# seungju-k1m/Distributed_RL

Hardware: NVIDIA H100
Metric: learner transitions/sec (sample+target+prio-update) (higher is better)
Workload: dtype f32

## Files before the change

distributed_rl_b200/csrc/gemm.cu:

```cuda
#include "common.cuh"
#include "hopper.cuh"
#include "operand_image.cuh"

namespace b2rl {
namespace gemm {

using namespace sm90;

constexpr int TM = 128, TN = 256, KC = image::KC;
constexpr int A_TILE = TM * 128, B_TILE = TN * 128;
constexpr int STAGE = 2 * A_TILE + 2 * B_TILE;
constexpr int STAGES = 2;
constexpr int CONSUMERS = 256;
constexpr int THREADS = CONSUMERS + 32;

template <bool TRANSPOSE>
__global__ void __launch_bounds__(256)
k_split_pack(const float* __restrict__ src, int src_rows, int src_cols, int64_t src_ld, int tile_rows,
             float* __restrict__ out, int rows_pad, int k_chunks, int row_off, int kc_off) {
  const int kc = blockIdx.y, row0 = blockIdx.x * 32;
  const int r = threadIdx.x >> 3, unit = threadIdx.x & 7;
  const int row = row0 + r;
  float v[4];
  if (TRANSPOSE) {
    __shared__ float tile[32][33];
    const int lane = threadIdx.x & 31, w = threadIdx.x >> 5;
#pragma unroll
    for (int j = 0; j < 4; ++j) {
      const int k = kc * KC + w * 4 + j, c = row0 + lane;
      tile[w * 4 + j][lane] = (k < src_rows && c < src_cols) ? src[(int64_t)k * src_ld + c] : 0.0f;
    }
    __syncthreads();
#pragma unroll
    for (int e = 0; e < 4; ++e) v[e] = tile[unit * 4 + e][r];
  } else {
    const int k = kc * KC + unit * 4;
    const float* p = src + (int64_t)row * src_ld + k;
    if (row < src_rows && k + 3 < src_cols && ((reinterpret_cast<uintptr_t>(p) & 15) == 0)) {
      const float4 q = *reinterpret_cast<const float4*>(p);
      v[0] = q.x; v[1] = q.y; v[2] = q.z; v[3] = q.w;
    } else {
#pragma unroll
      for (int e = 0; e < 4; ++e) v[e] = (row < src_rows && k + e < src_cols) ? p[e] : 0.0f;
    }
  }
  const int irow = row_off + row, ikc = kc_off + kc;
  if (irow >= rows_pad) return;
  image::store_unit(out, image::offset(irow, ikc, unit, tile_rows, rows_pad), image::term_stride(k_chunks, rows_pad), v);
}

constexpr int ACT_PAD = 1;

template <bool TRANSPOSE>
__global__ void __launch_bounds__(256)
k_pack_act_nhwc(const float* __restrict__ y, int B, int HW, int C, int relu, float* __restrict__ out,
                int rows_pad, int k_chunks) {
  extern __shared__ float s_act[];
  const int K = C * HW;
  if (!TRANSPOSE) {
    const int b = blockIdx.x;
    const int ld = C + ACT_PAD;
    const uint32_t magic_c = (uint32_t)((0x100000000ull + C - 1) / C);
    const uint32_t magic_hw = (uint32_t)((0x100000000ull + HW - 1) / HW);
    if (b < B) {
      const float* src = y + (int64_t)b * K;
      for (int i = threadIdx.x; i < K; i += 256) {
        float v = src[i];
        if (relu) v = fmaxf(v, 0.0f);
        const int hw = (int)__umulhi((uint32_t)i, magic_c);
        s_act[hw * ld + (i - hw * C)] = v;
      }
    }
    __syncthreads();
    const int64_t ts = image::term_stride(k_chunks, rows_pad);
    for (int w = threadIdx.x; w < k_chunks * 8; w += 256) {
      const int kc = w >> 3, unit = w & 7;
      const int f0 = kc * KC + unit * 4;
      int c = (int)__umulhi((uint32_t)f0, magic_hw), hw = f0 - c * HW;
      float v[4];
#pragma unroll
      for (int e = 0; e < 4; ++e) {
        v[e] = (b < B && f0 + e < K) ? s_act[hw * ld + c] : 0.0f;
        if (++hw == HW) { hw = 0; ++c; }
      }
      image::store_unit(out, image::offset(b, kc, unit, TM, rows_pad), ts, v);
    }
  } else {
    const int kc = blockIdx.x, hw = blockIdx.y;
    const int ld = C + ACT_PAD;
    for (int i = threadIdx.x; i < 32 * C; i += 256) {
      const int bb = i / C, c = i - bb * C, b = kc * KC + bb;
      float v = (b < B) ? y[((int64_t)b * HW + hw) * C + c] : 0.0f;
      if (relu) v = fmaxf(v, 0.0f);
      s_act[bb * ld + c] = v;
    }
    __syncthreads();
    const int64_t ts = image::term_stride(k_chunks, rows_pad);
    for (int w = threadIdx.x; w < C * 8; w += 256) {
      const int c = w >> 3, unit = w & 7;
      float v[4];
#pragma unroll
      for (int e = 0; e < 4; ++e) v[e] = s_act[(unit * 4 + e) * ld + c];
      image::store_unit(out, image::offset(c * HW + hw, kc, unit, TN, rows_pad), ts, v);
    }
  }
}

__global__ void __launch_bounds__(256)
k_pack_zero_rows(float* __restrict__ out, int row0, int rows_pad, int k_chunks, int tile_rows) {
  const int64_t ts = image::term_stride(k_chunks, rows_pad);
  const int n_rows = rows_pad - row0;
  const int64_t total = (int64_t)n_rows * k_chunks * 8;
  const float zero[4] = {0.f, 0.f, 0.f, 0.f};
  for (int64_t w = (int64_t)blockIdx.x * 256 + threadIdx.x; w < total; w += (int64_t)gridDim.x * 256) {
    const int unit = (int)(w & 7);
    const int64_t q = w >> 3;
    const int kc = (int)(q / n_rows), f = row0 + (int)(q - (int64_t)kc * n_rows);
    image::store_unit(out, image::offset(f, kc, unit, tile_rows, rows_pad), ts, zero);
  }
}

__global__ void __launch_bounds__(256)
k_unflatten_relu_mask(const float* __restrict__ gx, int64_t gx_ld, int splits, int64_t split_stride,
                      const float* __restrict__ y, int HW, int C, float* __restrict__ out) {
  extern __shared__ float s_act[];
  const int b = blockIdx.x, K = C * HW;
  const float* gr = gx + (int64_t)b * gx_ld;
  for (int i = threadIdx.x; i < K; i += 256) {
    float v = gr[i];
    for (int z = 1; z < splits; ++z) v += gr[z * split_stride + i];
    s_act[i] = v;
  }
  __syncthreads();
  const float* yr = y + (int64_t)b * K;
  float* o = out + (int64_t)b * K;
  for (int i = threadIdx.x; i < K; i += 256) {
    const int hw = i / C, c = i - hw * C;
    o[i] = (yr[i] > 0.0f) ? s_act[c * HW + hw] : 0.0f;
  }
}

struct Params {
  const float* a;
  const float* b;
  float* c;
  int64_t M, N, ldc;
  int64_t m_tiles, n_tiles, k_chunks;
  int32_t splits;
};

__global__ void __launch_bounds__(THREADS, 1)
k_gemm_tf32x3(const __grid_constant__ Params P) {
  extern __shared__ __align__(1024) uint8_t smem_raw[];
  uint8_t* smem = smem_raw + ((1024u - (sptr(smem_raw) & 1023u)) & 1023u);
  __shared__ __align__(8) uint64_t full[STAGES], empty[STAGES];
  const int warp = threadIdx.x >> 5, lane = threadIdx.x & 31;
  const int64_t mt = blockIdx.x, nt = blockIdx.y;
  const int64_t per = (P.k_chunks + P.splits - 1) / P.splits;
  const int64_t k0 = (int64_t)blockIdx.z * per;
  const int64_t k1 = (k0 + per < P.k_chunks) ? k0 + per : P.k_chunks;
  const int64_t nk = k1 - k0;

  if (threadIdx.x == 0) {
    for (int i = 0; i < STAGES; ++i) { mbar_init(&full[i], 1); mbar_init(&empty[i], CONSUMERS); }
    mbar_init_fence();
  }
  __syncthreads();
  if (nk <= 0) return;

  if (warp == CONSUMERS / 32) {
    if (lane == 0) {
      const int64_t a_term = P.k_chunks * P.m_tiles * (TM * 32);
      const int64_t b_term = P.k_chunks * P.n_tiles * (TN * 32);
      for (int64_t i = 0; i < nk; ++i) {
        const int s = (int)(i % STAGES);
        mbar_wait(&empty[s], ((i / STAGES) & 1) ^ 1);
        const int64_t kc = k0 + i;
        const float* a_hi = P.a + (kc * P.m_tiles + mt) * (TM * 32);
        const float* b_hi = P.b + (kc * P.n_tiles + nt) * (TN * 32);
        uint8_t* st = smem + (size_t)s * STAGE;
        mbar_expect_tx(&full[s], STAGE);
        bulk_g2s(st, a_hi, A_TILE, &full[s]);
        bulk_g2s(st + A_TILE, a_hi + a_term, A_TILE, &full[s]);
        bulk_g2s(st + 2 * A_TILE, b_hi, B_TILE, &full[s]);
        bulk_g2s(st + 2 * A_TILE + B_TILE, b_hi + b_term, B_TILE, &full[s]);
      }
    }
    return;
  }

  const int wg = warp >> 2;
  float acc[128];
  for (int64_t i = 0; i < nk; ++i) {
    const int s = (int)(i % STAGES);
    mbar_wait(&full[s], (i / STAGES) & 1);
    const uint32_t base = sptr(smem + (size_t)s * STAGE);
    const uint32_t a_hi = base + wg * (64 * 128), a_lo = a_hi + A_TILE, b_hi = base + 2 * A_TILE, b_lo = b_hi + B_TILE;
    wg_fence();
#pragma unroll
    for (int ks = 0; ks < 4; ++ks) {
      const uint32_t o = ks * 32;
      mma_tf32_n256(acc, make_desc(a_lo + o), make_desc(b_hi + o), (i | ks) ? 1u : 0u);
      mma_tf32_n256(acc, make_desc(a_hi + o), make_desc(b_lo + o), 1u);
      mma_tf32_n256(acc, make_desc(a_hi + o), make_desc(b_hi + o), 1u);
    }
    wg_commit();
    wg_wait<1>();
    wg_fence_regs(acc);
    if (i > 0) mbar_arrive(&empty[(i - 1) % STAGES]);
  }
  wg_wait<0>();
  wg_fence_regs(acc);
  const int64_t r0 = mt * TM + wg * 64 + (warp & 3) * 16 + (lane >> 2);
  float* cz = P.c + (int64_t)blockIdx.z * P.M * P.ldc;
#pragma unroll
  for (int j = 0; j < TN / 8; ++j) {
    const int64_t n = nt * TN + 8 * j + 2 * (lane & 3);
#pragma unroll
    for (int h = 0; h < 2; ++h) {
      const int64_t m = r0 + 8 * h;
      if (m >= P.M || n >= P.N) continue;
      float* dst = cz + m * P.ldc + n;
      if (n + 1 < P.N) *reinterpret_cast<float2*>(dst) = make_float2(acc[4 * j + 2 * h], acc[4 * j + 2 * h + 1]);
      else dst[0] = acc[4 * j + 2 * h];
    }
  }
}

__global__ void __launch_bounds__(256)
k_splitk_reduce(const float* __restrict__ partial, int splits, int64_t M, int64_t N, int64_t ldc, float* __restrict__ c) {
  const int64_t q = (int64_t)blockIdx.x * blockDim.x + threadIdx.x;
  const int64_t per_row = ldc >> 2;
  if (q >= M * per_row) return;
  const int64_t m = q / per_row, n = (q - m * per_row) << 2;
  if (n >= N) return;
  const int64_t off = m * ldc + n, stride = M * ldc;
  if (n + 3 < N) {
    float4 a = *reinterpret_cast<const float4*>(partial + off);
    for (int z = 1; z < splits; ++z) {
      const float4 b = *reinterpret_cast<const float4*>(partial + z * stride + off);
      a.x += b.x; a.y += b.y; a.z += b.z; a.w += b.w;
    }
    *reinterpret_cast<float4*>(c + off) = a;
  } else {
    for (int e = 0; n + e < N; ++e) {
      float a = partial[off + e];
      for (int z = 1; z < splits; ++z) a += partial[z * stride + off + e];
      c[off + e] = a;
    }
  }
}

}
}

using namespace b2rl;

extern "C" int64_t b2rl_gemm_packed_floats(int64_t rows, int64_t k, int32_t b_role) {
  const int64_t tr = b_role ? gemm::TN : gemm::TM;
  const int64_t rows_pad = (rows + tr - 1) / tr * tr, kc = (k + gemm::KC - 1) / gemm::KC;
  return 2 * rows_pad * kc * gemm::KC;
}

extern "C" int b2rl_gemm_split_pack_into(const float* src_dev, int64_t src_rows, int64_t src_cols, int64_t src_ld,
                                         int32_t transpose, int32_t b_role, float* out_dev, int64_t total_rows,
                                         int64_t total_k, int64_t row_offset, int64_t k_offset, void* stream) {
  B2RL_REQUIRE(src_dev && out_dev, "null argument");
  B2RL_REQUIRE(src_rows >= 1 && src_cols >= 1 && src_ld >= src_cols, "bad shape");
  B2RL_REQUIRE(((uintptr_t)out_dev % 16) == 0, "packed operand must be 16-byte aligned");
  const int64_t rows = transpose ? src_cols : src_rows, k = transpose ? src_rows : src_cols;
  B2RL_REQUIRE(row_offset >= 0 && k_offset >= 0 && row_offset + rows <= total_rows && k_offset + k <= total_k,
               "piece outside the operand");
  B2RL_REQUIRE(row_offset % 32 == 0 && k_offset % gemm::KC == 0, "piece offsets must be multiples of 32");
  B2RL_REQUIRE((rows % 32 == 0 || row_offset + rows == total_rows) && (k % gemm::KC == 0 || k_offset + k == total_k),
               "an inner piece must be a multiple of 32 rows / 32 contraction elements");
  const int tr = b_role ? gemm::TN : gemm::TM;
  const int64_t rows_pad = (total_rows + tr - 1) / tr * tr, kc_total = (total_k + gemm::KC - 1) / gemm::KC;
  B2RL_REQUIRE(rows_pad < (1 << 30) && kc_total <= 65535, "operand too large");
  const int64_t rows_cover = (row_offset + rows == total_rows) ? rows_pad - row_offset : rows;
  const int64_t kc_cover = (k + gemm::KC - 1) / gemm::KC;
  dim3 grid((unsigned)(rows_cover / 32), (unsigned)kc_cover);
  if (transpose)
    gemm::k_split_pack<true><<<grid, 256, 0, (cudaStream_t)stream>>>(src_dev, (int)src_rows, (int)src_cols, src_ld, tr,
                                                                     out_dev, (int)rows_pad, (int)kc_total,
                                                                     (int)row_offset, (int)(k_offset / gemm::KC));
  else
    gemm::k_split_pack<false><<<grid, 256, 0, (cudaStream_t)stream>>>(src_dev, (int)src_rows, (int)src_cols, src_ld, tr,
                                                                      out_dev, (int)rows_pad, (int)kc_total,
                                                                      (int)row_offset, (int)(k_offset / gemm::KC));
  count_launch();
  B2RL_CHECK_LAUNCH();
  return B2RL_OK;
}

extern "C" int b2rl_gemm_split_pack(const float* src_dev, int64_t src_rows, int64_t src_cols, int64_t src_ld,
                                    int32_t transpose, int32_t b_role, float* out_dev, void* stream) {
  const int64_t rows = transpose ? src_cols : src_rows, k = transpose ? src_rows : src_cols;
  return b2rl_gemm_split_pack_into(src_dev, src_rows, src_cols, src_ld, transpose, b_role, out_dev, rows, k, 0, 0, stream);
}

constexpr int64_t MAX_CHUNKS_PER_SPLIT = 32;

static int64_t gemm_splits(int64_t M, int64_t N, int64_t K, int sms) {
  const int64_t tiles = ((M + gemm::TM - 1) / gemm::TM) * ((N + gemm::TN - 1) / gemm::TN);
  const int64_t kc = (K + gemm::KC - 1) / gemm::KC;
  int64_t splits = sms / (tiles > 0 ? tiles : 1);
  if (splits < 1) splits = 1;
  if (splits > kc) splits = kc;
  if (splits * MAX_CHUNKS_PER_SPLIT < kc) splits = (kc + MAX_CHUNKS_PER_SPLIT - 1) / MAX_CHUNKS_PER_SPLIT;
  const int64_t per = (kc + splits - 1) / splits;
  return (kc + per - 1) / per;
}

static int gemm_sms(int* out) {
  int dev = 0;
  B2RL_CUDA(cudaGetDevice(&dev));
  B2RL_CUDA(sm_count(dev, out));
  return B2RL_OK;
}

extern "C" int64_t b2rl_gemm_workspace_floats(int64_t M, int64_t N, int64_t K, int64_t ldc) {
  int sms = 0;
  if (gemm_sms(&sms) != B2RL_OK) return -1;
  const int64_t splits = gemm_splits(M, N, K, sms);
  return splits > 1 ? splits * M * ldc : 0;
}

static int gemm_launch(const float* a_packed_dev, const float* b_packed_dev, float* out, int64_t M, int64_t N,
                       int64_t K, int64_t ldc, int64_t splits, cudaStream_t st) {
  int dev = 0;
  B2RL_CUDA(cudaGetDevice(&dev));
  const size_t smem_bytes = (size_t)gemm::STAGES * gemm::STAGE + 1024;
  B2RL_CUDA(set_max_dynamic_smem<gemm::k_gemm_tf32x3>(dev, smem_bytes));
  gemm::Params P{};
  P.a = a_packed_dev; P.b = b_packed_dev;
  P.c = out;
  P.M = M; P.N = N; P.ldc = ldc;
  P.m_tiles = (M + gemm::TM - 1) / gemm::TM;
  P.n_tiles = (N + gemm::TN - 1) / gemm::TN;
  P.k_chunks = (K + gemm::KC - 1) / gemm::KC;
  P.splits = (int32_t)splits;
  dim3 grid((unsigned)P.m_tiles, (unsigned)P.n_tiles, (unsigned)splits);
  gemm::k_gemm_tf32x3<<<grid, gemm::THREADS, smem_bytes, st>>>(P);
  count_launch();
  B2RL_CHECK_LAUNCH();
  return B2RL_OK;
}

extern "C" int b2rl_gemm_tf32x3_partials(const float* a_packed_dev, const float* b_packed_dev, float* partials_dev,
                                         int64_t M, int64_t N, int64_t K, int64_t ldc, void* stream) {
  B2RL_REQUIRE(a_packed_dev && b_packed_dev && partials_dev, "null argument");
  B2RL_REQUIRE(M >= 1 && N >= 1 && K >= 1 && ldc >= N, "bad shape");
  B2RL_REQUIRE(((uintptr_t)partials_dev % 16) == 0 && (ldc % 4) == 0,
               "partials must be 16-byte aligned with ldc % 4 == 0");
  int sms = 0;
  if (int rc = gemm_sms(&sms)) return rc;
  return gemm_launch(a_packed_dev, b_packed_dev, partials_dev, M, N, K, ldc, gemm_splits(M, N, K, sms),
                     (cudaStream_t)stream);
}

extern "C" int b2rl_gemm_tf32x3(const float* a_packed_dev, const float* b_packed_dev, float* c_dev, int64_t M,
                                int64_t N, int64_t K, int64_t ldc, float* workspace_dev, void* stream) {
  B2RL_REQUIRE(a_packed_dev && b_packed_dev && c_dev, "null argument");
  B2RL_REQUIRE(M >= 1 && N >= 1 && K >= 1 && ldc >= N, "bad shape");
  B2RL_REQUIRE(((uintptr_t)c_dev % 16) == 0 && (ldc % 4) == 0, "C must be 16-byte aligned with ldc % 4 == 0");
  int sms = 0;
  if (int rc = gemm_sms(&sms)) return rc;
  const int64_t splits = gemm_splits(M, N, K, sms);
  B2RL_REQUIRE(splits == 1 || (workspace_dev && ((uintptr_t)workspace_dev % 16) == 0),
               "this shape splits K: pass b2rl_gemm_workspace_floats() floats of 16-byte aligned workspace");
  cudaStream_t st = (cudaStream_t)stream;
  if (int rc = gemm_launch(a_packed_dev, b_packed_dev, splits > 1 ? workspace_dev : c_dev, M, N, K, ldc, splits, st))
    return rc;
  if (splits > 1) {
    const int64_t quads = M * (ldc >> 2);
    gemm::k_splitk_reduce<<<(unsigned)((quads + 255) / 256), 256, 0, st>>>(workspace_dev, (int)splits, M, N, ldc, c_dev);
    count_launch();
    B2RL_CHECK_LAUNCH();
  }
  return B2RL_OK;
}


extern "C" int b2rl_gemm_pack_act_nhwc(const float* y_dev, int64_t B, int64_t HW, int64_t C, int32_t relu, int32_t transpose,
                                       float* out_dev, void* stream) {
  B2RL_REQUIRE(y_dev && out_dev, "null argument");
  B2RL_REQUIRE(B >= 1 && HW >= 1 && C >= 1 && C * HW < (1 << 24) && B < (1 << 24), "bad shape");
  B2RL_REQUIRE(((uintptr_t)out_dev % 16) == 0, "packed operand must be 16-byte aligned");
  const int64_t K = C * HW;
  cudaStream_t st = (cudaStream_t)stream;
  if (!transpose) {
    const int64_t rows_pad = (B + gemm::TM - 1) / gemm::TM * gemm::TM, kc = (K + gemm::KC - 1) / gemm::KC;
    const size_t smem = (size_t)HW * (C + gemm::ACT_PAD) * sizeof(float);
    B2RL_REQUIRE(smem <= 48 * 1024, "activation row too large for the staging tile");
    gemm::k_pack_act_nhwc<false><<<(unsigned)rows_pad, 256, smem, st>>>(y_dev, (int)B, (int)HW, (int)C, relu, out_dev,
                                                                       (int)rows_pad, (int)kc);
    count_launch();
  } else {
    const int64_t rows_pad = (K + gemm::TN - 1) / gemm::TN * gemm::TN, kc = (B + gemm::KC - 1) / gemm::KC;
    const size_t smem = (size_t)32 * (C + gemm::ACT_PAD) * sizeof(float);
    B2RL_REQUIRE(smem <= 48 * 1024 && HW <= 65535, "activation tile too large");
    gemm::k_pack_act_nhwc<true><<<dim3((unsigned)kc, (unsigned)HW), 256, smem, st>>>(y_dev, (int)B, (int)HW, (int)C, relu,
                                                                                    out_dev, (int)rows_pad, (int)kc);
    count_launch();
    if (rows_pad > K) {
      gemm::k_pack_zero_rows<<<64, 256, 0, st>>>(out_dev, (int)K, (int)rows_pad, (int)kc, gemm::TN);
      count_launch();
    }
  }
  B2RL_CHECK_LAUNCH();
  return B2RL_OK;
}

extern "C" int b2rl_unflatten_relu_mask(const float* gx_dev, int64_t gx_ld, int32_t splits, int64_t split_stride,
                                        const float* y_dev, int64_t B, int64_t HW, int64_t C, float* out_dev,
                                        void* stream) {
  B2RL_REQUIRE(gx_dev && y_dev && out_dev, "null argument");
  B2RL_REQUIRE(B >= 1 && HW >= 1 && C >= 1 && gx_ld >= C * HW, "bad shape");
  B2RL_REQUIRE(splits >= 1 && (splits == 1 || split_stride >= B * gx_ld), "bad split-K partials");
  const size_t smem = (size_t)C * HW * sizeof(float);
  B2RL_REQUIRE(smem <= 48 * 1024, "activation row too large for the staging tile");
  gemm::k_unflatten_relu_mask<<<(unsigned)B, 256, smem, (cudaStream_t)stream>>>(gx_dev, gx_ld, splits, split_stride,
                                                                              y_dev, (int)HW, (int)C, out_dev);
  count_launch();
  B2RL_CHECK_LAUNCH();
  return B2RL_OK;
}
```

distributed_rl_b200/csrc/hopper.cuh:

```cuda
#pragma once
#include <stdint.h>

namespace b2rl {
namespace sm90 {

__device__ __forceinline__ uint32_t sptr(const void* p) { return (uint32_t)__cvta_generic_to_shared(p); }
__device__ __forceinline__ void mbar_init(uint64_t* b, uint32_t c) {
  asm volatile("mbarrier.init.shared::cta.b64 [%0], %1;" ::"r"(sptr(b)), "r"(c));
}
__device__ __forceinline__ void mbar_init_fence() {
  asm volatile("fence.mbarrier_init.release.cluster;" ::: "memory");
  asm volatile("fence.proxy.async.shared::cta;" ::: "memory");
}
__device__ __forceinline__ void mbar_expect_tx(uint64_t* b, uint32_t bytes) {
  asm volatile("mbarrier.arrive.expect_tx.shared::cta.b64 _, [%0], %1;" ::"r"(sptr(b)), "r"(bytes) : "memory");
}
__device__ __forceinline__ void mbar_arrive(uint64_t* b) {
  asm volatile("mbarrier.arrive.shared::cta.b64 _, [%0];" ::"r"(sptr(b)) : "memory");
}
__device__ __forceinline__ void mbar_wait(uint64_t* b, uint32_t parity) {
  asm volatile(
      "{\n\t.reg .pred p;\n\t"
      "W_%=:\n\t"
      "mbarrier.try_wait.parity.shared::cta.b64 p, [%0], %1;\n\t"
      "@p bra D_%=;\n\t"
      "bra W_%=;\n\t"
      "D_%=:\n\t}" ::"r"(sptr(b)), "r"(parity) : "memory");
}
__device__ __forceinline__ void bulk_g2s(void* dst, const void* src, uint32_t bytes, uint64_t* bar) {
  asm volatile("cp.async.bulk.shared::cluster.global.mbarrier::complete_tx::bytes [%0], [%1], %2, [%3];" ::"r"(
                   sptr(dst)), "l"(src), "r"(bytes), "r"(sptr(bar)) : "memory");
}
__device__ __forceinline__ void bulk_s2g(void* dst, const void* src, uint32_t bytes) {
  asm volatile("cp.async.bulk.global.shared::cta.bulk_group [%0], [%1], %2;" ::"l"(dst), "r"(sptr(src)), "r"(bytes)
               : "memory");
}
__device__ __forceinline__ void bulk_commit() { asm volatile("cp.async.bulk.commit_group;" ::: "memory"); }
template <int N>
__device__ __forceinline__ void bulk_wait_read() { asm volatile("cp.async.bulk.wait_group.read %0;" ::"n"(N) : "memory"); }
__device__ __forceinline__ void bulk_wait_all() { asm volatile("cp.async.bulk.wait_group 0;" ::: "memory"); }
__device__ __forceinline__ void fence_async_smem() { asm volatile("fence.proxy.async.shared::cta;" ::: "memory"); }
__device__ __forceinline__ void named_sync(int id, int threads) {
  asm volatile("bar.sync %0, %1;" ::"r"(id), "r"(threads) : "memory");
}

__device__ __forceinline__ uint64_t make_desc(uint32_t smem_addr) {
  return (uint64_t)((smem_addr & 0x3FFFFu) >> 4) | (1ull << 16) | ((uint64_t)(1024 >> 4) << 32) | (1ull << 62);
}

__device__ __forceinline__ void wg_fence() { asm volatile("wgmma.fence.sync.aligned;" ::: "memory"); }
__device__ __forceinline__ void wg_commit() { asm volatile("wgmma.commit_group.sync.aligned;" ::: "memory"); }
template <int N>
__device__ __forceinline__ void wg_wait() { asm volatile("wgmma.wait_group.sync.aligned %0;" ::"n"(N) : "memory"); }
template <typename T, int R>
__device__ __forceinline__ void wg_fence_regs(T (&d)[R]) {
#pragma unroll
  for (int i = 0; i < R; ++i) asm volatile("" : "+r"(reinterpret_cast<uint32_t&>(d[i]))::"memory");
}

__device__ __forceinline__ void mma_tf32_n256(float (&d)[128], uint64_t a, uint64_t b, uint32_t accumulate) {
  asm volatile(
      "{\n\t.reg .pred p;\n\tsetp.ne.b32 p, %130, 0;\n\t"
      "wgmma.mma_async.sync.aligned.m64n256k8.f32.tf32.tf32 {%0,%1,%2,%3,%4,%5,%6,%7,%8,%9,%10,%11,%12,%13,%14,%15,%16,%17,%18,%19,%20,%21,%22,%23,%24,%25,%26,%27,%28,%29,%30,%31,%32,%33,%34,%35,%36,%37,%38,%39,%40,%41,%42,%43,%44,%45,%46,%47,%48,%49,%50,%51,%52,%53,%54,%55,%56,%57,%58,%59,%60,%61,%62,%63,%64,%65,%66,%67,%68,%69,%70,%71,%72,%73,%74,%75,%76,%77,%78,%79,%80,%81,%82,%83,%84,%85,%86,%87,%88,%89,%90,%91,%92,%93,%94,%95,%96,%97,%98,%99,%100,%101,%102,%103,%104,%105,%106,%107,%108,%109,%110,%111,%112,%113,%114,%115,%116,%117,%118,%119,%120,%121,%122,%123,%124,%125,%126,%127}, %128, %129, p, 1, 1;\n\t}"
      : "+f"(d[0]), "+f"(d[1]), "+f"(d[2]), "+f"(d[3]), "+f"(d[4]), "+f"(d[5]), "+f"(d[6]), "+f"(d[7]), "+f"(d[8]), "+f"(d[9]), "+f"(d[10]), "+f"(d[11]), "+f"(d[12]), "+f"(d[13]), "+f"(d[14]), "+f"(d[15]), "+f"(d[16]), "+f"(d[17]), "+f"(d[18]), "+f"(d[19]), "+f"(d[20]), "+f"(d[21]), "+f"(d[22]), "+f"(d[23]), "+f"(d[24]), "+f"(d[25]), "+f"(d[26]), "+f"(d[27]), "+f"(d[28]), "+f"(d[29]), "+f"(d[30]), "+f"(d[31]), "+f"(d[32]), "+f"(d[33]), "+f"(d[34]), "+f"(d[35]), "+f"(d[36]), "+f"(d[37]), "+f"(d[38]), "+f"(d[39]), "+f"(d[40]), "+f"(d[41]), "+f"(d[42]), "+f"(d[43]), "+f"(d[44]), "+f"(d[45]), "+f"(d[46]), "+f"(d[47]), "+f"(d[48]), "+f"(d[49]), "+f"(d[50]), "+f"(d[51]), "+f"(d[52]), "+f"(d[53]), "+f"(d[54]), "+f"(d[55]), "+f"(d[56]), "+f"(d[57]), "+f"(d[58]), "+f"(d[59]), "+f"(d[60]), "+f"(d[61]), "+f"(d[62]), "+f"(d[63]), "+f"(d[64]), "+f"(d[65]), "+f"(d[66]), "+f"(d[67]), "+f"(d[68]), "+f"(d[69]), "+f"(d[70]), "+f"(d[71]), "+f"(d[72]), "+f"(d[73]), "+f"(d[74]), "+f"(d[75]), "+f"(d[76]), "+f"(d[77]), "+f"(d[78]), "+f"(d[79]), "+f"(d[80]), "+f"(d[81]), "+f"(d[82]), "+f"(d[83]), "+f"(d[84]), "+f"(d[85]), "+f"(d[86]), "+f"(d[87]), "+f"(d[88]), "+f"(d[89]), "+f"(d[90]), "+f"(d[91]), "+f"(d[92]), "+f"(d[93]), "+f"(d[94]), "+f"(d[95]), "+f"(d[96]), "+f"(d[97]), "+f"(d[98]), "+f"(d[99]), "+f"(d[100]), "+f"(d[101]), "+f"(d[102]), "+f"(d[103]), "+f"(d[104]), "+f"(d[105]), "+f"(d[106]), "+f"(d[107]), "+f"(d[108]), "+f"(d[109]), "+f"(d[110]), "+f"(d[111]), "+f"(d[112]), "+f"(d[113]), "+f"(d[114]), "+f"(d[115]), "+f"(d[116]), "+f"(d[117]), "+f"(d[118]), "+f"(d[119]), "+f"(d[120]), "+f"(d[121]), "+f"(d[122]), "+f"(d[123]), "+f"(d[124]), "+f"(d[125]), "+f"(d[126]), "+f"(d[127])
      : "l"(a), "l"(b), "r"(accumulate));
}

__device__ __forceinline__ void mma_u8s8_n128(int32_t (&d)[64], uint64_t a, uint64_t b, uint32_t accumulate) {
  asm volatile(
      "{\n\t.reg .pred p;\n\tsetp.ne.b32 p, %66, 0;\n\t"
      "wgmma.mma_async.sync.aligned.m64n128k32.s32.u8.s8 {%0,%1,%2,%3,%4,%5,%6,%7,%8,%9,%10,%11,%12,%13,%14,%15,%16,%17,%18,%19,%20,%21,%22,%23,%24,%25,%26,%27,%28,%29,%30,%31,%32,%33,%34,%35,%36,%37,%38,%39,%40,%41,%42,%43,%44,%45,%46,%47,%48,%49,%50,%51,%52,%53,%54,%55,%56,%57,%58,%59,%60,%61,%62,%63}, %64, %65, p;\n\t}"
      : "+r"(d[0]), "+r"(d[1]), "+r"(d[2]), "+r"(d[3]), "+r"(d[4]), "+r"(d[5]), "+r"(d[6]), "+r"(d[7]), "+r"(d[8]), "+r"(d[9]), "+r"(d[10]), "+r"(d[11]), "+r"(d[12]), "+r"(d[13]), "+r"(d[14]), "+r"(d[15]), "+r"(d[16]), "+r"(d[17]), "+r"(d[18]), "+r"(d[19]), "+r"(d[20]), "+r"(d[21]), "+r"(d[22]), "+r"(d[23]), "+r"(d[24]), "+r"(d[25]), "+r"(d[26]), "+r"(d[27]), "+r"(d[28]), "+r"(d[29]), "+r"(d[30]), "+r"(d[31]), "+r"(d[32]), "+r"(d[33]), "+r"(d[34]), "+r"(d[35]), "+r"(d[36]), "+r"(d[37]), "+r"(d[38]), "+r"(d[39]), "+r"(d[40]), "+r"(d[41]), "+r"(d[42]), "+r"(d[43]), "+r"(d[44]), "+r"(d[45]), "+r"(d[46]), "+r"(d[47]), "+r"(d[48]), "+r"(d[49]), "+r"(d[50]), "+r"(d[51]), "+r"(d[52]), "+r"(d[53]), "+r"(d[54]), "+r"(d[55]), "+r"(d[56]), "+r"(d[57]), "+r"(d[58]), "+r"(d[59]), "+r"(d[60]), "+r"(d[61]), "+r"(d[62]), "+r"(d[63])
      : "l"(a), "l"(b), "r"(accumulate));
}

__device__ __forceinline__ void mma_u8s8_n64(int32_t (&d)[32], uint64_t a, uint64_t b, uint32_t accumulate) {
  asm volatile(
      "{\n\t.reg .pred p;\n\tsetp.ne.b32 p, %34, 0;\n\t"
      "wgmma.mma_async.sync.aligned.m64n64k32.s32.u8.s8 {%0,%1,%2,%3,%4,%5,%6,%7,%8,%9,%10,%11,%12,%13,%14,%15,%16,%17,%18,%19,%20,%21,%22,%23,%24,%25,%26,%27,%28,%29,%30,%31}, %32, %33, p;\n\t}"
      : "+r"(d[0]), "+r"(d[1]), "+r"(d[2]), "+r"(d[3]), "+r"(d[4]), "+r"(d[5]), "+r"(d[6]), "+r"(d[7]), "+r"(d[8]), "+r"(d[9]), "+r"(d[10]), "+r"(d[11]), "+r"(d[12]), "+r"(d[13]), "+r"(d[14]), "+r"(d[15]), "+r"(d[16]), "+r"(d[17]), "+r"(d[18]), "+r"(d[19]), "+r"(d[20]), "+r"(d[21]), "+r"(d[22]), "+r"(d[23]), "+r"(d[24]), "+r"(d[25]), "+r"(d[26]), "+r"(d[27]), "+r"(d[28]), "+r"(d[29]), "+r"(d[30]), "+r"(d[31])
      : "l"(a), "l"(b), "r"(accumulate));
}

}
}
```

distributed_rl_b200/csrc/operand_image.cuh:

```cuda
#pragma once
#include <cstdint>

namespace b2rl {
namespace image {

constexpr int KC = 32;

__device__ __forceinline__ void split_tf32(float x, float& hi, float& lo) {
  const uint32_t u = __float_as_uint(x);
  uint32_t h = (u + 0x1000u) & 0xFFFFE000u;
  if ((h & 0x7F800000u) == 0x7F800000u) h = u & 0xFFFFE000u;
  hi = __uint_as_float(h);
  lo = ((u & 0x7F800000u) == 0x7F800000u) ? 0.0f : x - hi;
  if ((u & 0x7F800000u) == 0x7F800000u) hi = x;
}

__host__ __device__ __forceinline__ int64_t term_stride(int k_chunks, int rows_pad) {
  return (int64_t)k_chunks * rows_pad * KC;
}

__device__ __forceinline__ int64_t offset(int row, int kc, int unit, int tile_rows, int rows_pad) {
  const int rt = row / tile_rows, rr = row - rt * tile_rows;
  return (((int64_t)kc * (rows_pad / tile_rows) + rt) * tile_rows + rr) * KC + ((unit ^ (rr & 7)) << 2);
}

__device__ __forceinline__ void store_unit(float* __restrict__ img, int64_t off, int64_t ts, const float v[4]) {
  float hi[4], lo[4];
#pragma unroll
  for (int e = 0; e < 4; ++e) split_tf32(v[e], hi[e], lo[e]);
  *reinterpret_cast<float4*>(img + off) = make_float4(hi[0], hi[1], hi[2], hi[3]);
  *reinterpret_cast<float4*>(img + ts + off) = make_float4(lo[0], lo[1], lo[2], lo[3]);
}

}
}
```

distributed_rl_b200/csrc/optim.cu:

```cuda
#include "common.cuh"
#include "operand_image.cuh"

namespace b2rl {

constexpr int OPT_MAX_TENSORS = 24;
constexpr int OPT_THREADS = 256;
constexpr int OPT_PER_THREAD = 4;
constexpr int64_t OPT_CHUNK = (int64_t)OPT_THREADS * OPT_PER_THREAD;

struct OptTable {
  float* p[OPT_MAX_TENSORS];
  float* g[OPT_MAX_TENSORS];
  float* sq[OPT_MAX_TENSORS];
  float* ga[OPT_MAX_TENSORS];
  int64_t numel[OPT_MAX_TENSORS];
  int32_t block_start[OPT_MAX_TENSORS + 1];
  float* img_fwd[OPT_MAX_TENSORS];
  float* img_wt[OPT_MAX_TENSORS];
  int32_t cols[OPT_MAX_TENSORS];
  int32_t n_off[OPT_MAX_TENSORS];
  int32_t fwd_rows_pad[OPT_MAX_TENSORS], fwd_kc[OPT_MAX_TENSORS];
  int32_t wt_rows_pad[OPT_MAX_TENSORS], wt_kc[OPT_MAX_TENSORS];
  int32_t n_tensors;
};

__device__ __forceinline__ float rmsprop_elem(float p, float g, float& sq, float& ga, float lr, float alpha,
                                              float one_m_alpha, float eps, int centered) {
  sq = __fmaf_rn(one_m_alpha * g, g, sq * alpha);
  float avg;
  if (centered) {
    ga = __fmaf_rn(one_m_alpha, g - ga, ga);
    avg = __fsqrt_rn(__fmaf_rn(-ga, ga, sq));
  } else {
    avg = __fsqrt_rn(sq);
  }
  return p - lr * (g / (avg + eps));
}

__global__ void __launch_bounds__(OPT_THREADS)
k_rmsprop(const __grid_constant__ OptTable T, float lr, float alpha, float one_m_alpha, float eps, int centered,
          double* __restrict__ sumsq ) {
  __shared__ double s_part[OPT_THREADS / 32];
  int t = 0;
  while (t + 1 < T.n_tensors && (int)blockIdx.x >= T.block_start[t + 1]) ++t;
  const int64_t base = (int64_t)(blockIdx.x - T.block_start[t]) * OPT_CHUNK;
  const int64_t n = T.numel[t];
  float* __restrict__ P = T.p[t];
  float* __restrict__ G = T.g[t];
  float* __restrict__ SQ = T.sq[t];
  float* __restrict__ GA = T.ga[t];
  double acc = 0.0;
  if (T.img_fwd[t] || T.img_wt[t]) {
    __shared__ float tile[32][33];
    const int tiles_k = T.cols[t] / image::KC;
    const int bt = (int)(blockIdx.x - T.block_start[t]), rt = bt / tiles_k, kc = bt - rt * tiles_k;
    const int r = threadIdx.x >> 3, unit = threadIdx.x & 7;
    const int64_t i0 = (int64_t)(rt * 32 + r) * T.cols[t] + kc * image::KC + unit * 4;
    float4 p4 = *reinterpret_cast<const float4*>(P + i0);
    const float4 g4 = *reinterpret_cast<const float4*>(G + i0);
    float4 sq4 = *reinterpret_cast<const float4*>(SQ + i0);
    float4 ga4 = centered ? *reinterpret_cast<const float4*>(GA + i0) : make_float4(0.f, 0.f, 0.f, 0.f);
    float* pv = &p4.x;
    const float* gv = &g4.x;
    float* sqv = &sq4.x;
    float* gav = &ga4.x;
#pragma unroll
    for (int e = 0; e < 4; ++e) {
      pv[e] = rmsprop_elem(pv[e], gv[e], sqv[e], gav[e], lr, alpha, one_m_alpha, eps, centered);
      acc += (double)gv[e] * (double)gv[e];
    }
    *reinterpret_cast<float4*>(P + i0) = p4;
    *reinterpret_cast<float4*>(SQ + i0) = sq4;
    if (centered) *reinterpret_cast<float4*>(GA + i0) = ga4;
    *reinterpret_cast<float4*>(G + i0) = make_float4(0.f, 0.f, 0.f, 0.f);
    if (T.img_fwd[t]) {
      const int rows_pad = T.fwd_rows_pad[t];
      image::store_unit(T.img_fwd[t], image::offset(T.n_off[t] + rt * 32 + r, kc, unit, 256, rows_pad),
                        image::term_stride(T.fwd_kc[t], rows_pad), pv);
    }
    if (T.img_wt[t]) {
#pragma unroll
      for (int e = 0; e < 4; ++e) tile[r][unit * 4 + e] = pv[e];
      __syncthreads();
      float v[4];
#pragma unroll
      for (int e = 0; e < 4; ++e) v[e] = tile[unit * 4 + e][r];
      const int rows_pad = T.wt_rows_pad[t];
      image::store_unit(T.img_wt[t], image::offset(kc * image::KC + r, T.n_off[t] / image::KC + rt, unit, 256, rows_pad),
                        image::term_stride(T.wt_kc[t], rows_pad), v);
    }
  } else {
#pragma unroll
    for (int u = 0; u < OPT_PER_THREAD; ++u) {
      const int64_t i = base + (int64_t)u * OPT_THREADS + threadIdx.x;
      if (i < n) {
        const float g = G[i];
        float sq = SQ[i], ga = centered ? GA[i] : 0.0f;
        P[i] = rmsprop_elem(P[i], g, sq, ga, lr, alpha, one_m_alpha, eps, centered);
        SQ[i] = sq;
        if (centered) GA[i] = ga;
        G[i] = 0.0f;
        acc += (double)g * (double)g;
      }
    }
  }
  if (sumsq) {
#pragma unroll
    for (int o = 16; o > 0; o >>= 1) acc += __shfl_down_sync(0xffffffffu, acc, o);
    if ((threadIdx.x & 31) == 0) s_part[threadIdx.x >> 5] = acc;
    __syncthreads();
    if (threadIdx.x == 0) {
      double s = 0.0;
      for (int w = 0; w < OPT_THREADS / 32; ++w) s += s_part[w];
      atomicAdd(sumsq + t, s);
    }
  }
}

__global__ void k_grad_norm_finish(double* __restrict__ sumsq, int n, float* __restrict__ out) {
  if (threadIdx.x != 0 || blockIdx.x != 0) return;
  double s = 0.0;
  for (int i = 0; i < n; ++i) { s += sqrt(sumsq[i]); sumsq[i] = 0.0; }
  *out = (float)sqrt(s);
}

}

using namespace b2rl;

extern "C" int b2rl_rmsprop_step(float* const* params, float* const* grads, float* const* square_avg,
                                 float* const* grad_avg, const int64_t* numel, int32_t n_tensors, double lr,
                                 double alpha, double eps, int32_t centered, const int64_t* images,
                                 double* sumsq_scratch_dev, float* grad_norm_out_dev, void* stream) {
  B2RL_REQUIRE(n_tensors >= 1 && n_tensors <= OPT_MAX_TENSORS, "1..24 tensors");
  B2RL_REQUIRE(params && grads && square_avg && numel, "null argument");
  B2RL_REQUIRE(!centered || grad_avg, "centered RMSprop needs grad_avg");
  B2RL_REQUIRE(!grad_norm_out_dev || sumsq_scratch_dev,
               "the gradient norm needs a zero-initialised scratch of n_tensors doubles");
  OptTable T{};
  T.n_tensors = n_tensors;
  int64_t blocks = 0;
  for (int i = 0; i < n_tensors; ++i) {
    B2RL_REQUIRE(numel[i] >= 1 && params[i] && grads[i] && square_avg[i] && (!centered || grad_avg[i]),
                 "bad tensor entry");
    T.p[i] = params[i]; T.g[i] = grads[i]; T.sq[i] = square_avg[i]; T.ga[i] = centered ? grad_avg[i] : nullptr;
    T.numel[i] = numel[i];
    const int64_t* im = images ? images + 6 * i : nullptr;
    if (im && (im[0] || im[1])) {
      const int64_t rows = im[2], cols = im[3], total_n = im[4], n_off = im[5];
      B2RL_REQUIRE(rows >= 32 && cols >= 32 && rows % 32 == 0 && cols % 32 == 0 && rows * cols == numel[i] &&
                   n_off >= 0 && n_off % 32 == 0 && n_off + rows <= total_n && total_n < (1 << 30) &&
                   cols < (1 << 30), "image tensor: rows, cols and offsets must be multiples of 32 inside the stack");
      B2RL_REQUIRE(((uintptr_t)params[i] | (uintptr_t)grads[i] | (uintptr_t)square_avg[i] |
                    (uintptr_t)(centered ? grad_avg[i] : nullptr) | (uintptr_t)im[0] | (uintptr_t)im[1]) % 16 == 0,
                   "image tensor: 16-byte aligned arrays and images");
      T.img_fwd[i] = reinterpret_cast<float*>(im[0]);
      T.img_wt[i] = reinterpret_cast<float*>(im[1]);
      T.cols[i] = (int32_t)cols;
      T.n_off[i] = (int32_t)n_off;
      T.fwd_rows_pad[i] = (int32_t)((total_n + 255) / 256 * 256);
      T.fwd_kc[i] = (int32_t)(cols / image::KC);
      T.wt_rows_pad[i] = (int32_t)((cols + 255) / 256 * 256);
      T.wt_kc[i] = (int32_t)((total_n + image::KC - 1) / image::KC);
    }
    T.block_start[i] = (int32_t)blocks;
    blocks += (numel[i] + OPT_CHUNK - 1) / OPT_CHUNK;
  }
  T.block_start[n_tensors] = (int32_t)blocks;
  B2RL_REQUIRE(blocks < (1LL << 31), "too many elements");
  cudaStream_t st = (cudaStream_t)stream;
  k_rmsprop<<<(unsigned)blocks, OPT_THREADS, 0, st>>>(T, (float)lr, (float)alpha, (float)(1.0 - alpha), (float)eps,
                                                      centered, sumsq_scratch_dev);
  count_launch();
  if (grad_norm_out_dev) {
    k_grad_norm_finish<<<1, 32, 0, st>>>(sumsq_scratch_dev, n_tensors, grad_norm_out_dev);
    count_launch();
  }
  B2RL_CHECK_LAUNCH();
  return B2RL_OK;
}

extern "C" int b2rl_rmsprop_norm_finish(double* sumsq_scratch_dev, int32_t n_tensors, float* grad_norm_out_dev,
                                        void* stream) {
  B2RL_REQUIRE(sumsq_scratch_dev && grad_norm_out_dev, "null argument");
  B2RL_REQUIRE(n_tensors >= 1 && n_tensors <= OPT_MAX_TENSORS, "1..24 tensors");
  k_grad_norm_finish<<<1, 32, 0, (cudaStream_t)stream>>>(sumsq_scratch_dev, n_tensors, grad_norm_out_dev);
  count_launch();
  B2RL_CHECK_LAUNCH();
  return B2RL_OK;
}
```

Measured before the change: 663,900.

## Switch GEMM operand image to 64B-swizzled half-chunks with a deeper pipeline

Re-lays out the packed TF32 hi/lo operand image from 32-float K chunks with 128B swizzle to 16-float half-chunks with 64B swizzle, and updates every packer plus the optimizer's image writers to the new offset function. The GEMM now streams twice as many half-size stages through a 4-stage ring instead of 2, with a parameterised wgmma wait depth for releasing stages. The aim is more in-flight TMA loads and better overlap of loads with MMAs at the same shared-memory footprint. The cost is twice as many barrier round-trips and issue overhead per K chunk, and the new swizzle and descriptor encoding must match exactly or the results are wrong.

```diff
diff --git a/distributed_rl_b200/csrc/gemm.cu b/distributed_rl_b200/csrc/gemm.cu
--- a/distributed_rl_b200/csrc/gemm.cu
+++ b/distributed_rl_b200/csrc/gemm.cu
@@ -7,10 +7,13 @@
 
 using namespace sm90;
 
-constexpr int TM = 128, TN = 256, KC = image::KC;
-constexpr int A_TILE = TM * 128, B_TILE = TN * 128;
+constexpr int TM = 128, TN = 256;
+constexpr int KC = image::KC, KH = image::KH;
+constexpr int A_TILE = TM * KH * 4, B_TILE = TN * KH * 4;
 constexpr int STAGE = 2 * A_TILE + 2 * B_TILE;
-constexpr int STAGES = 2;
+constexpr int STAGES = 4;
+constexpr int WG_DEPTH = 1;
+static_assert(WG_DEPTH >= 0 && WG_DEPTH < STAGES, "a released stage must not be one the MMAs still read");
 constexpr int CONSUMERS = 256;
 constexpr int THREADS = CONSUMERS + 32;
 
@@ -46,7 +49,8 @@
   }
   const int irow = row_off + row, ikc = kc_off + kc;
   if (irow >= rows_pad) return;
-  image::store_unit(out, image::offset(irow, ikc, unit, tile_rows, rows_pad), image::term_stride(k_chunks, rows_pad), v);
+  image::store_unit(out, image::offset(irow, ikc * KC + unit * 4, tile_rows, rows_pad), image::term_stride(k_chunks, rows_pad),
+                    v);
 }
 
 constexpr int ACT_PAD = 1;
@@ -83,7 +87,7 @@
         v[e] = (b < B && f0 + e < K) ? s_act[hw * ld + c] : 0.0f;
         if (++hw == HW) { hw = 0; ++c; }
       }
-      image::store_unit(out, image::offset(b, kc, unit, TM, rows_pad), ts, v);
+      image::store_unit(out, image::offset(b, f0, TM, rows_pad), ts, v);
     }
   } else {
     const int kc = blockIdx.x, hw = blockIdx.y;
@@ -101,7 +105,7 @@
       float v[4];
 #pragma unroll
       for (int e = 0; e < 4; ++e) v[e] = s_act[(unit * 4 + e) * ld + c];
-      image::store_unit(out, image::offset(c * HW + hw, kc, unit, TN, rows_pad), ts, v);
+      image::store_unit(out, image::offset(c * HW + hw, kc * KC + unit * 4, TN, rows_pad), ts, v);
     }
   }
 }
@@ -116,7 +120,7 @@
     const int unit = (int)(w & 7);
     const int64_t q = w >> 3;
     const int kc = (int)(q / n_rows), f = row0 + (int)(q - (int64_t)kc * n_rows);
-    image::store_unit(out, image::offset(f, kc, unit, tile_rows, rows_pad), ts, zero);
+    image::store_unit(out, image::offset(f, kc * KC + unit * 4, tile_rows, rows_pad), ts, zero);
   }
 }
 
@@ -159,7 +163,7 @@
   const int64_t per = (P.k_chunks + P.splits - 1) / P.splits;
   const int64_t k0 = (int64_t)blockIdx.z * per;
   const int64_t k1 = (k0 + per < P.k_chunks) ? k0 + per : P.k_chunks;
-  const int64_t nk = k1 - k0;
+  const int64_t nk = 2 * (k1 - k0);
 
   if (threadIdx.x == 0) {
     for (int i = 0; i < STAGES; ++i) { mbar_init(&full[i], 1); mbar_init(&empty[i], CONSUMERS); }
@@ -170,14 +174,14 @@
 
   if (warp == CONSUMERS / 32) {
     if (lane == 0) {
-      const int64_t a_term = P.k_chunks * P.m_tiles * (TM * 32);
-      const int64_t b_term = P.k_chunks * P.n_tiles * (TN * 32);
+      const int64_t a_term = P.k_chunks * P.m_tiles * (TM * KC);
+      const int64_t b_term = P.k_chunks * P.n_tiles * (TN * KC);
       for (int64_t i = 0; i < nk; ++i) {
         const int s = (int)(i % STAGES);
         mbar_wait(&empty[s], ((i / STAGES) & 1) ^ 1);
-        const int64_t kc = k0 + i;
-        const float* a_hi = P.a + (kc * P.m_tiles + mt) * (TM * 32);
-        const float* b_hi = P.b + (kc * P.n_tiles + nt) * (TN * 32);
+        const int64_t kh = 2 * k0 + i;
+        const float* a_hi = P.a + (kh * P.m_tiles + mt) * (TM * KH);
+        const float* b_hi = P.b + (kh * P.n_tiles + nt) * (TN * KH);
         uint8_t* st = smem + (size_t)s * STAGE;
         mbar_expect_tx(&full[s], STAGE);
         bulk_g2s(st, a_hi, A_TILE, &full[s]);
@@ -191,23 +195,24 @@
 
   const int wg = warp >> 2;
   float acc[128];
+#pragma unroll 1
   for (int64_t i = 0; i < nk; ++i) {
     const int s = (int)(i % STAGES);
     mbar_wait(&full[s], (i / STAGES) & 1);
     const uint32_t base = sptr(smem + (size_t)s * STAGE);
-    const uint32_t a_hi = base + wg * (64 * 128), a_lo = a_hi + A_TILE, b_hi = base + 2 * A_TILE, b_lo = b_hi + B_TILE;
+    const uint32_t a_hi = base + wg * (64 * KH * 4), a_lo = a_hi + A_TILE, b_hi = base + 2 * A_TILE, b_lo = b_hi + B_TILE;
     wg_fence();
 #pragma unroll
-    for (int ks = 0; ks < 4; ++ks) {
+    for (int ks = 0; ks < KH / 8; ++ks) {
       const uint32_t o = ks * 32;
-      mma_tf32_n256(acc, make_desc(a_lo + o), make_desc(b_hi + o), (i | ks) ? 1u : 0u);
-      mma_tf32_n256(acc, make_desc(a_hi + o), make_desc(b_lo + o), 1u);
-      mma_tf32_n256(acc, make_desc(a_hi + o), make_desc(b_hi + o), 1u);
+      mma_tf32_n256(acc, make_desc_sw64(a_lo + o), make_desc_sw64(b_hi + o), (i | ks) ? 1u : 0u);
+      mma_tf32_n256(acc, make_desc_sw64(a_hi + o), make_desc_sw64(b_lo + o), 1u);
+      mma_tf32_n256(acc, make_desc_sw64(a_hi + o), make_desc_sw64(b_hi + o), 1u);
     }
     wg_commit();
-    wg_wait<1>();
+    wg_wait<WG_DEPTH>();
     wg_fence_regs(acc);
-    if (i > 0) mbar_arrive(&empty[(i - 1) % STAGES]);
+    if (i >= WG_DEPTH) mbar_arrive(&empty[(i - WG_DEPTH) % STAGES]);
   }
   wg_wait<0>();
   wg_fence_regs(acc);
diff --git a/distributed_rl_b200/csrc/hopper.cuh b/distributed_rl_b200/csrc/hopper.cuh
--- a/distributed_rl_b200/csrc/hopper.cuh
+++ b/distributed_rl_b200/csrc/hopper.cuh
@@ -47,6 +47,9 @@
 __device__ __forceinline__ uint64_t make_desc(uint32_t smem_addr) {
   return (uint64_t)((smem_addr & 0x3FFFFu) >> 4) | (1ull << 16) | ((uint64_t)(1024 >> 4) << 32) | (1ull << 62);
 }
+__device__ __forceinline__ uint64_t make_desc_sw64(uint32_t smem_addr) {
+  return (uint64_t)((smem_addr & 0x3FFFFu) >> 4) | (1ull << 16) | ((uint64_t)(512 >> 4) << 32) | (2ull << 62);
+}
 
 __device__ __forceinline__ void wg_fence() { asm volatile("wgmma.fence.sync.aligned;" ::: "memory"); }
 __device__ __forceinline__ void wg_commit() { asm volatile("wgmma.commit_group.sync.aligned;" ::: "memory"); }
diff --git a/distributed_rl_b200/csrc/operand_image.cuh b/distributed_rl_b200/csrc/operand_image.cuh
--- a/distributed_rl_b200/csrc/operand_image.cuh
+++ b/distributed_rl_b200/csrc/operand_image.cuh
@@ -5,6 +5,7 @@
 namespace image {
 
 constexpr int KC = 32;
+constexpr int KH = 16;
 
 __device__ __forceinline__ void split_tf32(float x, float& hi, float& lo) {
   const uint32_t u = __float_as_uint(x);
@@ -19,9 +20,10 @@
   return (int64_t)k_chunks * rows_pad * KC;
 }
 
-__device__ __forceinline__ int64_t offset(int row, int kc, int unit, int tile_rows, int rows_pad) {
+__device__ __forceinline__ int64_t offset(int row, int k, int tile_rows, int rows_pad) {
   const int rt = row / tile_rows, rr = row - rt * tile_rows;
-  return (((int64_t)kc * (rows_pad / tile_rows) + rt) * tile_rows + rr) * KC + ((unit ^ (rr & 7)) << 2);
+  const int kh = k / KH, unit = (k / 4) & 3;
+  return (((int64_t)kh * (rows_pad / tile_rows) + rt) * tile_rows + rr) * KH + ((unit ^ ((rr >> 1) & 3)) << 2);
 }
 
 __device__ __forceinline__ void store_unit(float* __restrict__ img, int64_t off, int64_t ts, const float v[4]) {
diff --git a/distributed_rl_b200/csrc/optim.cu b/distributed_rl_b200/csrc/optim.cu
--- a/distributed_rl_b200/csrc/optim.cu
+++ b/distributed_rl_b200/csrc/optim.cu
@@ -75,7 +75,7 @@
     *reinterpret_cast<float4*>(G + i0) = make_float4(0.f, 0.f, 0.f, 0.f);
     if (T.img_fwd[t]) {
       const int rows_pad = T.fwd_rows_pad[t];
-      image::store_unit(T.img_fwd[t], image::offset(T.n_off[t] + rt * 32 + r, kc, unit, 256, rows_pad),
+      image::store_unit(T.img_fwd[t], image::offset(T.n_off[t] + rt * 32 + r, kc * image::KC + unit * 4, 256, rows_pad),
                         image::term_stride(T.fwd_kc[t], rows_pad), pv);
     }
     if (T.img_wt[t]) {
@@ -86,7 +86,7 @@
 #pragma unroll
       for (int e = 0; e < 4; ++e) v[e] = tile[unit * 4 + e][r];
       const int rows_pad = T.wt_rows_pad[t];
-      image::store_unit(T.img_wt[t], image::offset(kc * image::KC + r, T.n_off[t] / image::KC + rt, unit, 256, rows_pad),
+      image::store_unit(T.img_wt[t], image::offset(kc * image::KC + r, T.n_off[t] + rt * 32 + unit * 4, 256, rows_pad),
                         image::term_stride(T.wt_kc[t], rows_pad), v);
     }
   } else {
```

Measured after the change: 686,600 (median of 6 runs). 3.4% higher.
